# PatrizioPerugini/depth_completion_MT

Hardware: AMD Instinct MI355X
Metric: depth frames/sec at 1216x352 (KITTI); achieved HBM GB/s vs peak (higher is better)
Workload: dtype f32

## Files before the change

### depth_completion_mt_amd/csrc/dcmt_kernels_fp_q16.h

```cpp
#pragma once

#include "dcmt_kernels_pair.h"
#include "median_pk3_nets.h"

namespace dcmt {

typedef unsigned short us2v __attribute__((ext_vector_type(2)));
__device__ __forceinline__ unsigned qmax(unsigned a, unsigned b)
{
    return __builtin_bit_cast(unsigned, __builtin_elementwise_max(__builtin_bit_cast(us2v, a), __builtin_bit_cast(us2v, b)));
}
__device__ __forceinline__ unsigned qmin(unsigned a, unsigned b)
{
    return __builtin_bit_cast(unsigned, __builtin_elementwise_min(__builtin_bit_cast(us2v, a), __builtin_bit_cast(us2v, b)));
}
__device__ __forceinline__ unsigned umax2(unsigned a, unsigned b) { return a > b ? a : b; }

typedef _Float16 hf2v __attribute__((ext_vector_type(2)));
__device__ __forceinline__ unsigned hmax2(unsigned a, unsigned b)
{
    return __builtin_bit_cast(unsigned, __builtin_elementwise_maximum(__builtin_bit_cast(hf2v, a), __builtin_bit_cast(hf2v, b)));
}
__device__ __forceinline__ unsigned hmin2(unsigned a, unsigned b)
{
    return __builtin_bit_cast(unsigned, __builtin_elementwise_minimum(__builtin_bit_cast(hf2v, a), __builtin_bit_cast(hf2v, b)));
}
__device__ __forceinline__ unsigned hmax3(unsigned a, unsigned b, unsigned c)
{
    return __builtin_bit_cast(unsigned, __builtin_elementwise_maximum(__builtin_elementwise_maximum(__builtin_bit_cast(hf2v, a), __builtin_bit_cast(hf2v, b)), __builtin_bit_cast(hf2v, c)));
}
__device__ __forceinline__ unsigned hmin3(unsigned a, unsigned b, unsigned c)
{
    return __builtin_bit_cast(unsigned, __builtin_elementwise_minimum(__builtin_elementwise_minimum(__builtin_bit_cast(hf2v, a), __builtin_bit_cast(hf2v, b)), __builtin_bit_cast(hf2v, c)));
}

__device__ __forceinline__ unsigned u_left(unsigned v) { return (unsigned)__builtin_amdgcn_update_dpp(0, (int)v, 0x138 , 0xf, 0xf, true); }
__device__ __forceinline__ unsigned u_right(unsigned v) { return (unsigned)__builtin_amdgcn_update_dpp(0, (int)v, 0x130 , 0xf, 0xf, true); }
__device__ __forceinline__ unsigned u_row_shr1(unsigned v) { return (unsigned)__builtin_amdgcn_update_dpp(0, (int)v, 0x111, 0xf, 0xf, true); }
__device__ __forceinline__ unsigned u_row_shl1(unsigned v) { return (unsigned)__builtin_amdgcn_update_dpp(0, (int)v, 0x101, 0xf, 0xf, true); }
__device__ __forceinline__ unsigned u_row_ror8(unsigned v) { return (unsigned)__builtin_amdgcn_update_dpp(0, (int)v, 0x128, 0xf, 0xf, true); }
__device__ __forceinline__ void u_row_scans4(unsigned a, unsigned b, unsigned& pa, unsigned& sa, unsigned& pb, unsigned& sb)
{
#define DCMT_U4(N) "v_max_u32_dpp %0, %0, %0 row_shr:" #N " row_mask:0xf bank_mask:0xf\n\t" \
                   "v_max_u32_dpp %1, %1, %1 row_shl:" #N " row_mask:0xf bank_mask:0xf\n\t" \
                   "v_max_u32_dpp %2, %2, %2 row_shr:" #N " row_mask:0xf bank_mask:0xf\n\t" \
                   "v_max_u32_dpp %3, %3, %3 row_shl:" #N " row_mask:0xf bank_mask:0xf\n\t"
    asm("s_nop 1\n\t"
        "v_max_u32_dpp %0, %4, %4 row_shr:1 row_mask:0xf bank_mask:0xf bound_ctrl:1\n\t"
        "v_max_u32_dpp %1, %4, %4 row_shl:1 row_mask:0xf bank_mask:0xf bound_ctrl:1\n\t"
        "v_max_u32_dpp %2, %5, %5 row_shr:1 row_mask:0xf bank_mask:0xf bound_ctrl:1\n\t"
        "v_max_u32_dpp %3, %5, %5 row_shl:1 row_mask:0xf bank_mask:0xf bound_ctrl:1\n\t"
        DCMT_U4(2) DCMT_U4(4)
        "v_max_u32_dpp %0, %0, %0 row_shr:8 row_mask:0xf bank_mask:0xf\n\t"
        "v_max_u32_dpp %1, %1, %1 row_shl:8 row_mask:0xf bank_mask:0xf\n\t" : "=&v"(pa), "=&v"(sa), "=&v"(pb), "=&v"(sb) : "v"(a), "v"(b));
#undef DCMT_U4
}

#define DCMT_QCX(a, b)   { const unsigned lo_ = qmin(v[a], v[b]); v[b] = qmax(v[a], v[b]); v[a] = lo_; }
#define DCMT_QCMIN(a, b) { v[a] = qmin(v[a], v[b]); }
#define DCMT_QCMAX(a, b) { v[b] = qmax(v[a], v[b]); }
__device__ __forceinline__ unsigned xor3(unsigned a, unsigned b, unsigned c) { return __builtin_amdgcn_bitop3_b32(a, b, c, 0x96); }
__device__ __forceinline__ void q_sort5(unsigned (&v)[5])
{
    const unsigned a = hmin3(v[0], v[1], v[2]), c = hmax3(v[0], v[1], v[2]), t = xor3(v[0], v[1], v[2]), b = xor3(t, a, c);
    const unsigned d = hmin2(v[3], v[4]), e = hmax2(v[3], v[4]);
    const unsigned s0 = hmin2(a, d), s4 = hmax2(c, e);
    const unsigned s1 = hmin3(hmax2(a, d), b, e), s3 = hmax3(hmin2(c, e), b, d);
    const unsigned s2 = xor3(xor3(t, v[3], v[4]), xor3(s0, s1, s3), s4);
    v[0] = s0; v[1] = s1; v[2] = s2; v[3] = s3; v[4] = s4;
}
__device__ __forceinline__ void q_merge55(const unsigned (&a)[5], const unsigned (&b)[5], unsigned (&P)[10])
{
    constexpr int out[10] = DCMT_MERGE55_OUT;
    unsigned v[10];
#pragma unroll
    for (int k = 0; k < 5; ++k) { v[k] = a[k]; v[5 + k] = b[k]; }
    DCMT_MERGE55_NET(DCMT_QCX, DCMT_QCMIN, DCMT_QCMAX)
#pragma unroll
    for (int k = 0; k < 10; ++k) P[k] = v[out[k]];
}
__device__ __forceinline__ void q_mid20(const unsigned (&pa)[10], const unsigned (&pb)[10], unsigned (&C)[6])
{
#define DCMT_IN_(k) ((k) < 10 ? pa[(k) < 10 ? (k) : 0] : pb[(k) >= 10 ? (k) - 10 : 0])
#define DCMT_OUT_(k) C[k]
    DCMT_MID20_PK3(DCMT_IN_, DCMT_OUT_)
#undef DCMT_IN_
#undef DCMT_OUT_
}
#undef DCMT_QCX
#undef DCMT_QCMIN
#undef DCMT_QCMAX
__device__ __forceinline__ unsigned q_final6(const unsigned (&C)[6], const unsigned (&a)[5])
{
    const unsigned m0 = hmax2(a[0], C[4]), m1 = hmax2(a[1], C[3]), m2 = hmax2(a[2], C[2]), m3 = hmax2(a[3], C[1]), m4 = hmax2(a[4], C[0]);
    return hmin2(hmin3(C[5], m0, m1), hmin3(m2, m3, m4));
}
struct MedianColumnQ {
    unsigned SE[4][5], SO[5], P[2][10], C[6];
    __device__ __forceinline__ void init()
    {
#pragma unroll
        for (int q = 0; q < 4; ++q)
#pragma unroll
            for (int k = 0; k < 5; ++k) SE[q][k] = 0;
#pragma unroll
        for (int k = 0; k < 5; ++k) SO[k] = 0;
#pragma unroll
        for (int k = 0; k < 10; ++k) { P[0][k] = 0; P[1][k] = 0; }
#pragma unroll
        for (int k = 0; k < 6; ++k) C[k] = 0;
    }
    template <int PP>
    __device__ __forceinline__ unsigned step(const unsigned (&s)[5])
    {
        unsigned m;
        if constexpr ((PP & 1) == 0) {
            constexpr int qs = (PP >> 1) & 3;
            q_merge55(SO, s, P[(PP >> 1) & 1]);
            q_mid20(P[((PP >> 1) + 1) & 1], P[(PP >> 1) & 1], C);
            m = q_final6(C, SE[(qs + 2) & 3]);
#pragma unroll
            for (int k = 0; k < 5; ++k) SE[qs][k] = s[k];
        } else {
            m = q_final6(C, s);
#pragma unroll
            for (int k = 0; k < 5; ++k) SO[k] = s[k];
        }
        return m;
    }
};

struct FpQ {
    static constexpr int H = 4;
    static constexpr int VW = 128 - 2 * H;
};

template <bool BLUR>
struct PostPipeP {
    F2 G1[8], MR[8];
    F2 last_out;
    FrameBuf of;
    unsigned ob;
    int rows, cols, gx, rle, rlo;
    bool outlane, edge_strip, outside;
    float max_depth, thr;

    __device__ __forceinline__ void init(float* out_frame, int rows_, int cols_, int gx0, int lane, float max_depth_, float thr_)
    {
        of.init(out_frame, (size_t)rows_ * cols_); rows = rows_; cols = cols_; max_depth = max_depth_; thr = thr_;
        gx = gx0 + 2 * lane;
        ob = 4u * (unsigned)min(max(gx, 0), cols - 2);
        outside = gx < 0 || gx >= cols;
        outlane = !outside && 2 * lane >= FpQ::H && 2 * lane < 128 - FpQ::H;
        rle = (reflect101(gx, cols) - gx0) >> 1;
        rlo = (reflect101(gx + 1, cols) - 1 - gx0) >> 1;
        edge_strip = gx0 < 0 || gx0 + 127 >= cols;
        last_out = {0.f, 0.f};
#pragma unroll
        for (int q = 0; q < 8; ++q) { G1[q] = {0.f, 0.f}; MR[q] = {0.f, 0.f}; }
    }

    enum { BORDER = 0, INNER = 1 };

    template <int PP, int MODE = BORDER>
    __device__ __forceinline__ void after_median(float me, float mo, int u)
    {
        MR[(PP + 4) & 7] = {me, mo};
        if constexpr (BLUR) {
            F2 mf = {me, mo};
            if (edge_strip) {
                const float re = __shfl(me, rle, 64), ro = __shfl(mo, rlo, 64);
                if (outside) mf = {re, ro};
            }
            const float el = from_left(mf.e), ol = from_left(mf.o), er = from_right(mf.e), orr = from_right(mf.o);
            G1[(PP + 4) & 7] = {gauss_taps(mf.e, __fadd_rn(ol, mf.o), __fadd_rn(el, er)), gauss_taps(mf.o, __fadd_rn(mf.e, er), __fadd_rn(ol, orr))};
        }
        const int o = u - 6;
        if (MODE != BORDER || (unsigned)o < (unsigned)rows) {
            const F2 mo_ = MR[(PP + 2) & 7];
            auto finish = [&](F2 u1, F2 u2, F2 d1, F2 d2) {
                F2 val = mo_;
                if constexpr (BLUR) {
                    const F2 g0 = G1[(PP + 2) & 7];
                    const float ae = gauss_taps(g0.e, __fadd_rn(u1.e, d1.e), __fadd_rn(u2.e, d2.e));
                    const float ao = gauss_taps(g0.o, __fadd_rn(u1.o, d1.o), __fadd_rn(u2.o, d2.o));
                    if (mo_.e >= thr) val.e = ae;
                    if (mo_.o >= thr) val.o = ao;
                }
                val = {invert_valid(val.e, max_depth, thr), invert_valid(val.o, max_depth, thr)};
                st2(of, outlane ? ob : kDropOffset, o, cols, val);
                last_out = val;
            };
            const F2 g_p2 = G1[(PP + 4) & 7], g_p1 = G1[(PP + 3) & 7], g_0 = G1[(PP + 2) & 7], g_m1 = G1[(PP + 1) & 7], g_m2 = G1[PP];
            if (BLUR && MODE == BORDER && (o < 2 || o + 2 >= rows)) {
                finish(o >= 1 ? g_m1 : g_p1,
                       o >= 2 ? g_m2 : (o == 1 ? g_0 : g_p2),
                       o + 1 < rows ? g_p1 : g_m1,
                       o + 2 < rows ? g_p2 : (o + 2 == rows ? g_0 : g_m2));
            } else {
                finish(g_m1, g_m2, g_p1, g_p2);
            }
        }
    }

    template <int PP, int MODE = BORDER>
    __device__ __forceinline__ void after_median_codes(unsigned m, int u)
    {
        static_assert(BLUR, "exact only on grid values; the select of LO :184 is not in here");
        float ce = (float)(m & 0xffffu), co = (float)(m >> 16);
        if (edge_strip) {
            const float re = __shfl(ce, rle, 64), ro = __shfl(co, rlo, 64);
            if (outside) { ce = re; co = ro; }
        }
        const float s1 = __fadd_rn(from_left(co), co), s2 = __fadd_rn(ce, from_right(ce));
        const float ue = __fadd_rn(from_left(s2), s2), wo = __fadd_rn(from_right(s1), s1);
        G1[(PP + 4) & 7] = {__builtin_fmaf(__fadd_rn(ce, s1), 4.0f, ue), __builtin_fmaf(__fadd_rn(co, s2), 4.0f, wo)};
        const int o = u - 6;
        if (MODE != BORDER || (unsigned)o < (unsigned)rows) {
            const float top = __fadd_rn(max_depth, (float)Q16::OFFSET * 0.00390625f);
            auto finish = [&](F2 u1, F2 u2, F2 d1, F2 d2) {
                const F2 g0 = G1[(PP + 2) & 7];
                const float ne = __builtin_fmaf(g0.e, 6.0f, __builtin_fmaf(__fadd_rn(u1.e, d1.e), 4.0f, __fadd_rn(u2.e, d2.e)));
                const float no = __builtin_fmaf(g0.o, 6.0f, __builtin_fmaf(__fadd_rn(u1.o, d1.o), 4.0f, __fadd_rn(u2.o, d2.o)));
                const F2 val = {__builtin_fmaf(ne, -0x1p-16f, top), __builtin_fmaf(no, -0x1p-16f, top)};
                st2(of, outlane ? ob : kDropOffset, o, cols, val);
                last_out = val;
            };
            const F2 g_p2 = G1[(PP + 4) & 7], g_p1 = G1[(PP + 3) & 7], g_0 = G1[(PP + 2) & 7], g_m1 = G1[(PP + 1) & 7], g_m2 = G1[PP];
            if (MODE == BORDER && (o < 2 || o + 2 >= rows)) {
                finish(o >= 1 ? g_m1 : g_p1,
                       o >= 2 ? g_m2 : (o == 1 ? g_0 : g_p2),
                       o + 1 < rows ? g_p1 : g_m1,
                       o + 2 < rows ? g_p2 : (o + 2 == rows ? g_0 : g_m2));
            } else {
                finish(g_m1, g_m2, g_p1, g_p2);
            }
        }
    }
};

#ifndef DCMT_FPQ_WAVES
#define DCMT_FPQ_WAVES 0
#endif
#ifndef DCMT_FPQ_PFD
#define DCMT_FPQ_PFD 6
#endif
template <bool BLUR, bool FILLED>
__global__ __launch_bounds__(256)
#if DCMT_FPQ_WAVES
__attribute__((amdgpu_waves_per_eu(DCMT_FPQ_WAVES, DCMT_FPQ_WAVES)))
#endif
void k_fp_q(const void* __restrict__ x6_, float* __restrict__ dst, int* __restrict__ counters,
            int rows_all, int cols, int strips, int batch, int xcd_map, float max_depth, float thr, const int* __restrict__ tb,
            int tbands)
{
    __shared__ unsigned s_delay[4][16 * (64 + 64 + 32)];
    const int lane = threadIdx.x & 63;
    const int wave = __builtin_amdgcn_readfirstlane(threadIdx.x >> 6);
    int f, strip;
    if (!wave_strip(blockIdx.x, wave, strips, batch, xcd_map, f, strip)) return;
    int* cnt = frame_counters(counters, f);
    const size_t fo = (size_t)f * rows_all * cols;
    const int gx0 = strip * FpQ::VW - FpQ::H;
    const int gxe = gx0 + 2 * lane;
    const int gxb = lane < 8 ? gx0 + 128 + 2 * lane : (lane < 16 ? gx0 + 128 + 2 * (lane - 8) + 1 :
                    (lane >= 56 ? gx0 - 16 + 2 * (lane - 56) : (lane >= 48 ? gx0 - 16 + 2 * (lane - 48) + 1 : gx0 + 128)));
    const int gxec = min(max(gxe, 0), cols - 2), gxoc = gxec + 1, gxbc = min(max(gxb, 0), cols - 1);
    int tie = 0, tio = 0, tib = 0, bie = rows_all - 1, bio = rows_all - 1, bib = rows_all - 1, V = 0;
    if (tb) {
        table_rows(tb, f, cols, tbands, rows_all, gxec, tie, bie);
        table_rows(tb, f, cols, tbands, rows_all, gxoc, tio, bio);
        table_rows(tb, f, cols, tbands, rows_all, gxbc, tib, bib);
        V = __builtin_amdgcn_readfirstlane(max(wave_min_i(min(min(tie, tio), tib)) - 8, 0));
    }
    const int rows = rows_all - V;
    constexpr unsigned EB = 2;
    FrameBuf sf;
    sf.init(reinterpret_cast<const float*>(static_cast<const char*>(x6_) + fo * EB), (size_t)rows_all * cols * EB / 4);
    const unsigned rowb = EB * (unsigned)cols;
    const unsigned sbe = EB * (unsigned)gxec + (unsigned)V * rowb, sbo = sbe + EB, sbb = EB * (unsigned)gxbc + (unsigned)V * rowb;
    const unsigned fle = EB * (unsigned)gxec + (unsigned)max(tie, V) * rowb, cee = EB * (unsigned)gxec + (unsigned)max(bie, V) * rowb;
    const unsigned flo = EB * (unsigned)gxoc + (unsigned)max(tio, V) * rowb, ceo = EB * (unsigned)gxoc + (unsigned)max(bio, V) * rowb;
    const unsigned flb = EB * (unsigned)gxbc + (unsigned)max(tib, V) * rowb, ceb = EB * (unsigned)gxbc + (unsigned)max(bib, V) * rowb;
    auto clamp3 = [](unsigned a, unsigned lo, unsigned hi) -> unsigned { unsigned r; asm("v_med3_u32 %0, %1, %2, %3" : "=v"(r) : "v"(a), "v"(lo), "v"(hi)); return r; };
    auto ld_code = [&](unsigned off) -> unsigned short { return (unsigned short)__builtin_amdgcn_raw_buffer_load_b16(sf.rs, off, 0, 0); };
    struct Raw { unsigned short e, o, b; };
    auto ld_row = [&](int row) -> Raw {
        return Raw{ld_code(clamp3(sbe + (unsigned)row * rowb, fle, cee)), ld_code(clamp3(sbo + (unsigned)row * rowb, flo, ceo)),
                   ld_code(clamp3(sbb + (unsigned)row * rowb, flb, ceb))};
    };
    auto pack = [](unsigned short e, unsigned short o) -> unsigned { return (unsigned)e | ((unsigned)o << 16); };
    const bool outside = gxe < 0 || gxe >= cols;
    const bool own = !outside && 2 * lane >= FpQ::H && 2 * lane < 128 - FpQ::H;
    const unsigned long long own_mask = __ballot(own);
    const bool edge_strip = gx0 < 0 || gx0 + 127 >= cols;
    const int rep_l = min(max((0 - gx0) >> 1, 0), 63), rep_r = min(max((cols - 2 - gx0) >> 1, 0), 63);
    const int a_m8 = ((lane - 8) & 63) * 4, a_p8 = ((lane + 8) & 63) * 4;
    const bool b_lo = lane < 8, b_hi = lane >= 56;
    unsigned* sd = s_delay[wave];
    unsigned (*dl_c)[64] = reinterpret_cast<unsigned (*)[64]>(sd);
    unsigned (*dl_a)[64] = reinterpret_cast<unsigned (*)[64]>(sd + 16 * 64);
    unsigned (*dl_b)[32] = reinterpret_cast<unsigned (*)[32]>(sd + 16 * 128);
    const int lb = lane < 16 ? lane : (lane >= 48 ? lane - 32 : 0);

    PostPipeP<BLUR> pipe;
    pipe.init(dst + fo + (size_t)V * cols, rows, cols, gx0, lane, max_depth, thr);
    MedianColumnQ mc;
    mc.init();

    const bool warm = V > 0;
    unsigned xa0 = 0, xb0 = 0;
    if (warm) { const Raw r = ld_row(0); xa0 = pack(r.e, r.o); xb0 = r.b; }
    unsigned short PFE[16], PFO[16], PFB[16];
    unsigned PFA[16], W2A[16], W6A[16], W2B[16], W6B[16];
#pragma unroll
    for (int q = 0; q < 16; ++q) { PFE[q] = PFO[q] = PFB[q] = 0; PFA[q] = 0; W2A[q] = W6A[q] = xa0; W2B[q] = W6B[q] = xb0; }
#pragma unroll
    for (int q = 0; q < 16; ++q) { dl_c[q][lane] = xa0; dl_a[q][lane] = xa0; dl_b[q][lb] = xb0; }
    constexpr int PFD = DCMT_FPQ_PFD;
#pragma unroll
    for (int q = 0; q < PFD; ++q) {
        const Raw r = ld_row(min(max(q + (warm ? 16 : 0) - 15, 0), rows - 1));
        PFE[q] = r.e; PFO[q] = r.o; PFB[q] = r.b;
    }
    unsigned vpa = xa0, vpb = xb0, x7_prev = xa0;
    int before = 0, after = 0;
    unsigned pend_v = xa0, pend_f1 = 0, pend_f2 = 0;
    unsigned long long pend_hme = 0, pend_hmo = 0;
    unsigned nxt_c = xa0, nxt_a = xa0, nxt_b = xb0;

    using Pipe = PostPipeP<BLUR>;
    using BorderMode = std::integral_constant<int, Pipe::BORDER>;
    auto fill_step = [&](auto P_, auto M_, int t) -> unsigned {
        constexpr int p = decltype(P_)::value;
        constexpr int MODE = decltype(M_)::value;
        unsigned xa;
        const unsigned xb = PFB[p];
        if constexpr (MODE == Pipe::BORDER) {
            xa = pack(PFE[p], PFO[p]);
            const Raw r = ld_row(min(max(t + PFD - 15, 0), rows - 1));
            PFE[(p + PFD) & 15] = r.e; PFO[(p + PFD) & 15] = r.o; PFB[(p + PFD) & 15] = r.b;
        } else {
            xa = PFA[p];
            const unsigned srow = (unsigned)(t + PFD - 15) * rowb;
            PFA[(p + PFD) & 15] = (unsigned)__builtin_amdgcn_raw_buffer_load_b32(sf.rs, sbe, srow, 0);
            PFB[(p + PFD) & 15] = (unsigned short)__builtin_amdgcn_raw_buffer_load_b16(sf.rs, sbb, srow, 0);
        }
        const int o = t - 31;
        unsigned x7 = pend_v;
        if ((pend_hme | pend_hmo) != 0ull) {
            const unsigned d = qmax(pend_f1, pend_f2);
            const bool he = __builtin_amdgcn_inverse_ballot_w64(pend_hme), ho = __builtin_amdgcn_inverse_ballot_w64(pend_hmo);
            const unsigned m = (he ? 0xffffu : 0u) | (ho ? 0xffff0000u : 0u);
            x7 = (d & m) | (pend_v & ~m);
            if (MODE != Pipe::BORDER || (unsigned)o < (unsigned)rows) {
                before += __builtin_popcountll(pend_hme & own_mask) + __builtin_popcountll(pend_hmo & own_mask);
                after += __builtin_popcountll(__builtin_amdgcn_ballot_w64((x7 << 16) <= Q16::HOLE_MAX_HI) & own_mask) +
                         __builtin_popcountll(__builtin_amdgcn_ballot_w64(x7 <= Q16::HOLE_MAX_HI) & own_mask);
            }
        }
        if (edge_strip) {
            const unsigned l0 = (unsigned)__shfl((int)x7, rep_l, 64), r0 = (unsigned)__shfl((int)x7, rep_r, 64);
            if (gxe < 0) x7 = (l0 & 0xffffu) | (l0 << 16);
            if (gxe >= cols) x7 = (r0 >> 16) | (r0 & 0xffff0000u);
        }
        if (MODE == Pipe::BORDER && o >= rows) { asm volatile("" ::); x7 = x7_prev; }
        x7_prev = x7;
        const unsigned w2a = hmax2(xa, vpa);
        vpa = xa;
        W2A[p] = w2a;
        const unsigned w6a = hmax3(w2a, W2A[(p + 14) & 15], W2A[(p + 12) & 15]);
        W6A[p] = w6a;
        const unsigned w18a = hmax3(w6a, W6A[(p + 10) & 15], W6A[(p + 4) & 15]);
        const unsigned v = nxt_c, w18a_old = nxt_a;
        nxt_c = dl_c[(p + 2) & 15][lane];
        nxt_a = dl_a[(p + 4) & 15][lane];
        dl_c[p][lane] = xa;
        dl_a[p][lane] = w18a;
        const unsigned w31a = hmax2(w18a, w18a_old);
        const unsigned w2b = hmax2(xb, vpb);
        vpb = xb;
        W2B[p] = w2b;
        const unsigned w6b = hmax3(w2b, W2B[(p + 14) & 15], W2B[(p + 12) & 15]);
        W6B[p] = w6b;
        const unsigned w18b = hmax3(w6b, W6B[(p + 10) & 15], W6B[(p + 4) & 15]);
        const unsigned w18b_old = nxt_b;
        nxt_b = dl_b[(p + 4) & 15][lb];
        dl_b[p][lb] = w18b;
        const unsigned w31b = hmax2(w18b, w18b_old);
        const unsigned long long vme = __builtin_amdgcn_ballot_w64((v << 16) <= Q16::HOLE_MAX_HI), vmo = __builtin_amdgcn_ballot_w64(v <= Q16::HOLE_MAX_HI);
        if ((vme | vmo) != 0ull) {
            const unsigned e = w31a & 0xffffu, od = w31a >> 16;
            const unsigned bo = u_row_ror8(w31b);
            unsigned pa, sa, pb, sb;
            u_row_scans4(umax2(e, od), umax2(w31b, bo), pa, sa, pb, sb);
            const unsigned px = u_row_shr1(lane < 7 ? pb : pa), sx = u_row_shl1(lane > 56 ? sb : sa);
            const unsigned so = umax2(b_hi ? bo : od, sx);
            const unsigned pe = umax2(b_lo ? w31b : e, px);
            pend_f1 = (unsigned)__builtin_amdgcn_ds_bpermute(a_m8, (int)(so | (sx << 16)));
            pend_f2 = (unsigned)__builtin_amdgcn_ds_bpermute(a_p8, (int)(px | (pe << 16)));
        }
        pend_v = v;
        pend_hme = vme; pend_hmo = vmo;
        return x7;
    };
    auto post_step = [&](auto PP_, auto M_, unsigned x, int u) {
        constexpr int PP = decltype(PP_)::value;
        constexpr int MODE = decltype(M_)::value;
        const unsigned rl = u_left(x), rr = u_right(x);
        unsigned s[5] = {rl, __builtin_amdgcn_alignbit(x, rl, 16), x, __builtin_amdgcn_alignbit(rr, x, 16), rr};
        q_sort5(s);
        const unsigned m = mc.template step<PP>(s);
        if constexpr (BLUR && FILLED) pipe.template after_median_codes<PP, MODE>(m, u);
        else pipe.template after_median<PP, MODE>(Q16::value(m & 0xffffu), Q16::value(m >> 16), u);
    };

    for (int t0 = warm ? 16 : 0; t0 < 32; t0 += 16) {
        static_for<0, 16>([&](auto P_) {
            constexpr int p = decltype(P_)::value;
            const unsigned x7 = fill_step(P_, BorderMode{}, t0 + p);
            if constexpr (p == 15) {
                if (t0 == 16) {
                    post_step(std::integral_constant<int, 0>{}, BorderMode{}, x7, 0);
                    post_step(std::integral_constant<int, 1>{}, BorderMode{}, x7, 1);
                    post_step(std::integral_constant<int, 2>{}, BorderMode{}, x7, 2);
                }
            }
        });
    }
    const int nsteps = rows + 35;
    int t0 = 32;
    auto main_step = [&](auto P_) {
        constexpr int p = decltype(P_)::value;
        const int t = t0 + p, u = t - 29;
        const unsigned x7 = fill_step(P_, BorderMode{}, t);
        post_step(std::integral_constant<int, ((p + 3) & 7)>{}, BorderMode{}, x7, u);
        if constexpr (p == 3) {
            if (t0 == 32 && V > 0) {
                FrameBuf top;
                top.init(dst + fo, (size_t)V * cols);
                const unsigned tbo = pipe.outlane ? pipe.ob : kDropOffset;
                for (int r = 0; r < V; ++r) st2(top, tbo, r, cols, pipe.last_out);
            }
        }
    };
    const int r_first = max(__builtin_amdgcn_readfirstlane(wave_max_i(max(max(tie, tio), tib))) - V, 0);
    const int r_last = min(__builtin_amdgcn_readfirstlane(wave_min_i(min(min(bie, bio), bib))) - V, rows - 1);
    auto interior = [&](int t) -> bool { return t >= 48 && t + PFD - 15 >= r_first && t + PFD <= r_last; };
    using InnerMode = std::integral_constant<int, Pipe::INNER>;
    for (; t0 < nsteps; t0 += 16) {
        if (interior(t0)) {
#pragma unroll
            for (int q = 0; q < PFD; ++q) PFA[q] = pack(PFE[q], PFO[q]);
            do {
                static_for<0, 16>([&](auto P_) {
                    constexpr int p = decltype(P_)::value;
                    int t = t0 + p;
                    asm volatile("" : "+s"(t));
                    const unsigned x7 = fill_step(P_, InnerMode{}, t);
                    post_step(std::integral_constant<int, ((p + 3) & 7)>{}, InnerMode{}, x7, t - 29);
                });
                t0 += 16;
            } while (interior(t0));
#pragma unroll
            for (int q = 0; q < PFD; ++q) { PFE[q] = (unsigned short)PFA[q]; PFO[q] = (unsigned short)(PFA[q] >> 16); }
        }
        static_for<0, 4>(main_step);
        if (t0 + 4 >= nsteps) break;
        static_for<4, 8>(main_step);
        if (t0 + 8 >= nsteps) break;
        static_for<8, 12>(main_step);
        if (t0 + 12 >= nsteps) break;
        static_for<12, 16>(main_step);
    }
    if (lane == 0) {
        if (before) atomicAdd(&cnt[0], before);
        if (after) atomicAdd(&cnt[1], after);
    }
}

}
```

Before: 770,600.

## Replace edge-strip shuffles with readlane fixes and add a halo-free fast scan path

Border reflection for edge strips now patches only the single reflected lane using readlane and inverse-ballot selects, replacing full-wave shuffles (ds_bpermute) on the input codes and median outputs. The reflect fix for median values moves from the post pipe into post_step on packed codes, so the pipe no longer carries the reflect-lane state. When no holes fall in the halo lanes, a cheaper 2-sequence DPP row scan replaces the 4-sequence cross-row scan. This cuts LDS permute traffic and DPP work in the inner loop, at the cost of more branching and exact-equivalence risk at the strip edges.

```diff
diff --git a/depth_completion_mt_amd/csrc/dcmt_kernels_fp_q16.h b/depth_completion_mt_amd/csrc/dcmt_kernels_fp_q16.h
--- a/depth_completion_mt_amd/csrc/dcmt_kernels_fp_q16.h
+++ b/depth_completion_mt_amd/csrc/dcmt_kernels_fp_q16.h
@@ -55,6 +55,19 @@
         "v_max_u32_dpp %1, %1, %1 row_shl:8 row_mask:0xf bank_mask:0xf\n\t" : "=&v"(pa), "=&v"(sa), "=&v"(pb), "=&v"(sb) : "v"(a), "v"(b));
 #undef DCMT_U4
 }
+__device__ __forceinline__ void u_row_scans2(unsigned a, unsigned& pa, unsigned& sa)
+{
+#define DCMT_U2(N) "s_nop 0\n\t" \
+                   "v_max_u32_dpp %0, %0, %0 row_shr:" #N " row_mask:0xf bank_mask:0xf\n\t" \
+                   "v_max_u32_dpp %1, %1, %1 row_shl:" #N " row_mask:0xf bank_mask:0xf\n\t"
+    asm("s_nop 1\n\t"
+        "v_max_u32_dpp %0, %2, %2 row_shr:1 row_mask:0xf bank_mask:0xf bound_ctrl:1\n\t"
+        "v_max_u32_dpp %1, %2, %2 row_shl:1 row_mask:0xf bank_mask:0xf bound_ctrl:1\n\t"
+        DCMT_U2(2) DCMT_U2(4) DCMT_U2(8) : "=&v"(pa), "=&v"(sa) : "v"(a));
+#undef DCMT_U2
+}
+__device__ __forceinline__ unsigned lane_get(unsigned v, int l) { return (unsigned)__builtin_amdgcn_readlane((int)v, l); }
+__device__ __forceinline__ unsigned lane_put(unsigned v, unsigned s, int l) { return __builtin_amdgcn_inverse_ballot_w64(1ull << l) ? s : v; }
 
 #define DCMT_QCX(a, b)   { const unsigned lo_ = qmin(v[a], v[b]); v[b] = qmax(v[a], v[b]); v[a] = lo_; }
 #define DCMT_QCMIN(a, b) { v[a] = qmin(v[a], v[b]); }
@@ -141,8 +154,8 @@
     F2 last_out;
     FrameBuf of;
     unsigned ob;
-    int rows, cols, gx, rle, rlo;
-    bool outlane, edge_strip, outside;
+    int rows, cols, gx;
+    bool outlane;
     float max_depth, thr;
 
     __device__ __forceinline__ void init(float* out_frame, int rows_, int cols_, int gx0, int lane, float max_depth_, float thr_)
@@ -150,11 +163,8 @@
         of.init(out_frame, (size_t)rows_ * cols_); rows = rows_; cols = cols_; max_depth = max_depth_; thr = thr_;
         gx = gx0 + 2 * lane;
         ob = 4u * (unsigned)min(max(gx, 0), cols - 2);
-        outside = gx < 0 || gx >= cols;
+        const bool outside = gx < 0 || gx >= cols;
         outlane = !outside && 2 * lane >= FpQ::H && 2 * lane < 128 - FpQ::H;
-        rle = (reflect101(gx, cols) - gx0) >> 1;
-        rlo = (reflect101(gx + 1, cols) - 1 - gx0) >> 1;
-        edge_strip = gx0 < 0 || gx0 + 127 >= cols;
         last_out = {0.f, 0.f};
 #pragma unroll
         for (int q = 0; q < 8; ++q) { G1[q] = {0.f, 0.f}; MR[q] = {0.f, 0.f}; }
@@ -167,11 +177,7 @@
     {
         MR[(PP + 4) & 7] = {me, mo};
         if constexpr (BLUR) {
-            F2 mf = {me, mo};
-            if (edge_strip) {
-                const float re = __shfl(me, rle, 64), ro = __shfl(mo, rlo, 64);
-                if (outside) mf = {re, ro};
-            }
+            const F2 mf = {me, mo};
             const float el = from_left(mf.e), ol = from_left(mf.o), er = from_right(mf.e), orr = from_right(mf.o);
             G1[(PP + 4) & 7] = {gauss_taps(mf.e, __fadd_rn(ol, mf.o), __fadd_rn(el, er)), gauss_taps(mf.o, __fadd_rn(mf.e, er), __fadd_rn(ol, orr))};
         }
@@ -207,11 +213,7 @@
     __device__ __forceinline__ void after_median_codes(unsigned m, int u)
     {
         static_assert(BLUR, "exact only on grid values; the select of LO :184 is not in here");
-        float ce = (float)(m & 0xffffu), co = (float)(m >> 16);
-        if (edge_strip) {
-            const float re = __shfl(ce, rle, 64), ro = __shfl(co, rlo, 64);
-            if (outside) { ce = re; co = ro; }
-        }
+        const float ce = (float)(m & 0xffffu), co = (float)(m >> 16);
         const float s1 = __fadd_rn(from_left(co), co), s2 = __fadd_rn(ce, from_right(ce));
         const float ue = __fadd_rn(from_left(s2), s2), wo = __fadd_rn(from_right(s1), s1);
         G1[(PP + 4) & 7] = {__builtin_fmaf(__fadd_rn(ce, s1), 4.0f, ue), __builtin_fmaf(__fadd_rn(co, s2), 4.0f, wo)};
@@ -293,10 +295,13 @@
     const bool outside = gxe < 0 || gxe >= cols;
     const bool own = !outside && 2 * lane >= FpQ::H && 2 * lane < 128 - FpQ::H;
     const unsigned long long own_mask = __ballot(own);
-    const bool edge_strip = gx0 < 0 || gx0 + 127 >= cols;
-    const int rep_l = min(max((0 - gx0) >> 1, 0), 63), rep_r = min(max((cols - 2 - gx0) >> 1, 0), 63);
+    const bool left_edge = gx0 < 0, right_edge = gx0 + 127 >= cols;
+    const bool edge_strip = left_edge || right_edge;
+    constexpr int lane_l = FpQ::H / 2 - 1;
+    const int lane_r = __builtin_amdgcn_readfirstlane(min(max((cols - gx0) >> 1, 3), 63));
     const int a_m8 = ((lane - 8) & 63) * 4, a_p8 = ((lane + 8) & 63) * 4;
     const bool b_lo = lane < 8, b_hi = lane >= 56;
+    const unsigned long long halo_holes = 0xff000000000000ffull & ~__ballot(outside);
     unsigned* sd = s_delay[wave];
     unsigned (*dl_c)[64] = reinterpret_cast<unsigned (*)[64]>(sd);
     unsigned (*dl_a)[64] = reinterpret_cast<unsigned (*)[64]>(sd + 16 * 64);
@@ -360,9 +365,8 @@
             }
         }
         if (edge_strip) {
-            const unsigned l0 = (unsigned)__shfl((int)x7, rep_l, 64), r0 = (unsigned)__shfl((int)x7, rep_r, 64);
-            if (gxe < 0) x7 = (l0 & 0xffffu) | (l0 << 16);
-            if (gxe >= cols) x7 = (r0 >> 16) | (r0 & 0xffff0000u);
+            if (left_edge) { const unsigned c = lane_get(x7, lane_l + 1); x7 = lane_put(x7, (c & 0xffffu) | (c << 16), lane_l); }
+            if (right_edge) { const unsigned c = lane_get(x7, lane_r - 1); x7 = lane_put(x7, (c >> 16) | (c & 0xffff0000u), lane_r); }
         }
         if (MODE == Pipe::BORDER && o >= rows) { asm volatile("" ::); x7 = x7_prev; }
         x7_prev = x7;
@@ -391,12 +395,21 @@
         const unsigned long long vme = __builtin_amdgcn_ballot_w64((v << 16) <= Q16::HOLE_MAX_HI), vmo = __builtin_amdgcn_ballot_w64(v <= Q16::HOLE_MAX_HI);
         if ((vme | vmo) != 0ull) {
             const unsigned e = w31a & 0xffffu, od = w31a >> 16;
-            const unsigned bo = u_row_ror8(w31b);
-            unsigned pa, sa, pb, sb;
-            u_row_scans4(umax2(e, od), umax2(w31b, bo), pa, sa, pb, sb);
-            const unsigned px = u_row_shr1(lane < 7 ? pb : pa), sx = u_row_shl1(lane > 56 ? sb : sa);
-            const unsigned so = umax2(b_hi ? bo : od, sx);
-            const unsigned pe = umax2(b_lo ? w31b : e, px);
+            unsigned px, sx, so, pe;
+            if (((vme | vmo) & halo_holes) != 0ull) {
+                const unsigned bo = u_row_ror8(w31b);
+                unsigned pa, sa, pb, sb;
+                u_row_scans4(umax2(e, od), umax2(w31b, bo), pa, sa, pb, sb);
+                px = u_row_shr1(lane < 7 ? pb : pa); sx = u_row_shl1(lane > 56 ? sb : sa);
+                so = umax2(b_hi ? bo : od, sx);
+                pe = umax2(b_lo ? w31b : e, px);
+            } else {
+                unsigned pa, sa;
+                u_row_scans2(umax2(e, od), pa, sa);
+                px = u_row_shr1(pa); sx = u_row_shl1(sa);
+                so = umax2(od, sx);
+                pe = umax2(e, px);
+            }
             pend_f1 = (unsigned)__builtin_amdgcn_ds_bpermute(a_m8, (int)(so | (sx << 16)));
             pend_f2 = (unsigned)__builtin_amdgcn_ds_bpermute(a_p8, (int)(px | (pe << 16)));
         }
@@ -410,7 +423,13 @@
         const unsigned rl = u_left(x), rr = u_right(x);
         unsigned s[5] = {rl, __builtin_amdgcn_alignbit(x, rl, 16), x, __builtin_amdgcn_alignbit(rr, x, 16), rr};
         q_sort5(s);
-        const unsigned m = mc.template step<PP>(s);
+        unsigned m = mc.template step<PP>(s);
+        if constexpr (BLUR) {
+            if (edge_strip) {
+                if (left_edge) m = lane_put(m, (lane_get(m, lane_l + 2) & 0xffffu) | (lane_get(m, lane_l + 1) & 0xffff0000u), lane_l);
+                if (right_edge) m = lane_put(m, (lane_get(m, lane_r - 1) & 0xffffu) | (lane_get(m, lane_r - 2) & 0xffff0000u), lane_r);
+            }
+        }
         if constexpr (BLUR && FILLED) pipe.template after_median_codes<PP, MODE>(m, u);
         else pipe.template after_median<PP, MODE>(Q16::value(m & 0xffffu), Q16::value(m >> 16), u);
     };
```

Measured after the change: 770,300 (median of 2 runs). Within noise of the previous version (-0.0%).
